# mindazhao/PWStableNet

Measured on AMD Instinct MI355X. Metric: stabilized frames/sec at 256x256 (netG fp32 + grid_sample), whole job, higher is better.
Workload: dtype f32

## Files before the change

### pwstablenet_amd/csrc/conv_ring_f32.hip

```cpp
#include "conv_common.h"

namespace pws {

typedef float rf_f32x2 __attribute__((ext_vector_type(2)));
typedef unsigned rf_u32x2 __attribute__((ext_vector_type(2)));

enum RingfMode {
    RF_K3S1 = 0,
    RF_CT4 = 1,
    RF_K3S2 = 2
};

struct RingfParams {
    const float *src_ptr[4];
    int src_c[4], src_ld[4];
    int nsrc;
    int N, H, W;
    int LH, LW;
    int OH, OW;
    int cout, cin_pad;
    const float *w;
    size_t w_bytes;
    const float *bias;
    int act;
    float *out;
    int out_ld;
    int tiles_x, tiles_y;
    unsigned ncob, ncls, nunits;
    int gpp;
};

template <int MODE_, int TH_, int R_, int NT_ = 2>
struct RfCfg {
    static constexpr int MODE = MODE_, TH = TH_, TW = 32, R = R_;
    static constexpr int NT = NT_, CO_UNIT = 32 * NT, WROWB = 128 * NT, WSL = 8 * NT;
    static_assert(NT == 1 || NT == 2, "output-channel blocks");
    static constexpr int KS = MODE == RF_K3S1 ? 3 : 2;
    static constexpr int TAPS = KS * KS;
    static constexpr int NPLANES = MODE == RF_K3S2 ? 4 : 1;
    static constexpr int NCLS = MODE == RF_CT4 ? 4 : 1;
    static constexpr int MWAVES = 8, LWAVES = 4, THREADS = 64 * (MWAVES + LWAVES);
    static_assert(TH == 16 || TH == 8, "tile");
    static constexpr int MT = TH / 8;
    static constexpr int IH = TH + KS - 1, IW = TW + KS - 1;
    static constexpr int CKG = 16;
    static constexpr int ROWB = CKG * 4;
    static constexpr int SPP = ROWB / 16;
    static constexpr int IN_SLOTS = IH * IW * SPP;
    static constexpr int IN_WI = (IN_SLOTS + 63) / 64;
    static constexpr int W_WI = TAPS * CKG * WROWB / 1024;
    static constexpr int NL = (IN_WI + W_WI + LWAVES - 1) / LWAVES;
    static constexpr int GROUP_BYTES = NL * LWAVES * 1024;
    static constexpr int W_OFF = IN_WI * 1024;
    static constexpr int LDS_BYTES = R * GROUP_BYTES;
    static constexpr int MIX_IT = IN_WI % LWAVES == 0 ? -1 : IN_WI / LWAVES;
    static_assert(LDS_BYTES <= 160 * 1024, "LDS");
    static_assert(R >= 2 && R <= 4, "ring depth");
    static_assert((R - 2) * NL <= 63, "vmcnt is 6 bits");
};

__device__ __forceinline__ void ringf_dma16(unsigned lds_addr, unsigned voff, __amdgpu_buffer_rsrc_t rsrc, unsigned soff) {
    unsigned keep;
    asm volatile("s_nop 4\n\ts_mov_b32 %0, m0\n\ts_mov_b32 m0, %1\n\ts_nop 0\n\tbuffer_load_dwordx4 %2, %3, %4 offen lds\n\ts_mov_b32 m0, %0"
                 : "=&s"(keep)
                 : "s"(lds_addr), "v"(voff), "s"(rsrc), "s"(soff));
}
__device__ __forceinline__ void ringf_dma16_m0(unsigned lds_addr, unsigned voff, __amdgpu_buffer_rsrc_t rsrc, unsigned soff) {
    asm volatile("s_nop 3\n\ts_mov_b32 m0, %0\n\ts_nop 0\n\tbuffer_load_dwordx4 %1, %2, %3 offen lds" ::"s"(lds_addr), "v"(voff), "s"(rsrc), "s"(soff));
}
template <int N>
__device__ __forceinline__ void ringf_wait_vmcnt() {
    asm volatile("s_waitcnt vmcnt(%0)" ::"n"(N) : "memory");
}
constexpr unsigned kRingfOob = 0x7ffffff0u;
__device__ __forceinline__ unsigned unif(unsigned v) { return __builtin_amdgcn_readfirstlane(v); }
__device__ __forceinline__ const char *unif(const char *ptr) {
    const unsigned long long a = reinterpret_cast<unsigned long long>(ptr);
    return reinterpret_cast<const char *>(((unsigned long long)unif((unsigned)(a >> 32)) << 32) | unif((unsigned)a));
}
template <class T>
__device__ __forceinline__ T selq4(const T (&a)[4], int i) {
    return i == 0 ? a[0] : (i == 1 ? a[1] : (i == 2 ? a[2] : a[3]));
}

struct RingfUnit {
    int n0, y0, x0, co0, py, px;
};
__device__ __forceinline__ RingfUnit ringf_unit(const RingfParams &p, unsigned u, int co_unit) {
    RingfUnit r;
    const unsigned cls = u % p.ncls, rest = u / p.ncls;
    const unsigned cob = rest % p.ncob, tile = rest / p.ncob;
    const unsigned tx = tile % (unsigned)p.tiles_x, t2 = tile / (unsigned)p.tiles_x;
    const unsigned ty = t2 % (unsigned)p.tiles_y;
    r.n0 = (int)(t2 / (unsigned)p.tiles_y);
    r.y0 = (int)ty, r.x0 = (int)tx, r.co0 = (int)cob * co_unit, r.py = (int)(cls >> 1), r.px = (int)(cls & 1);
    return r;
}

template <class C>
__global__ void __launch_bounds__(C::THREADS, 3) conv_ringf_kernel(const RingfParams p) {
    extern __shared__ __attribute__((aligned(16))) unsigned char lds[];
    const int tid = threadIdx.x, lane = tid & 63;
    const int wv = __builtin_amdgcn_readfirstlane(tid >> 6);
    const int l31 = lane & 31, hi = lane >> 5;

    const unsigned G = gridDim.x;
    const unsigned nxc = G < (unsigned)kXcds ? G : (unsigned)kXcds;
    const unsigned xcd = blockIdx.x % nxc, slot = blockIdx.x / nxc;
    const unsigned nx = G / nxc + (xcd < G % nxc ? 1u : 0u);
    const unsigned c_begin = (unsigned)((unsigned long long)xcd * p.nunits / nxc);
    const unsigned c_end = (unsigned)((unsigned long long)(xcd + 1) * p.nunits / nxc);
    if (c_begin + slot >= c_end) return;
    const unsigned u_begin = c_begin + slot, u_end = c_end, u_step = nx;
    const unsigned my_units = (u_end - u_begin + u_step - 1) / u_step;
    const int ngroups = C::NPLANES * p.gpp;
    const unsigned total = my_units * (unsigned)ngroups;

    if (wv >= C::MWAVES) {
        const int lw = wv - C::MWAVES;
        int ia[C::NL], ib[C::NL];
#pragma unroll
        for (int it = 0; it < C::NL; ++it) {
            const int wi = it * C::LWAVES + lw;
            const int j = wi * 64 + lane;
            if (wi < C::IN_WI) {
                const int q = j / C::SPP, sp = j % C::SPP;
                const int lx = q % C::IW, ly = q / C::IW;
                ia[it] = j < C::IN_SLOTS ? (ly << 10 | lx) : -1;
                ib[it] = (sp ^ ((lx >> 2) & 3)) * 16;
            } else if (wi < C::IN_WI + C::W_WI) {
                const int jj = j - C::IN_WI * 64;
                ia[it] = jj / C::WSL;
                ib[it] = jj % C::WSL;
            } else {
                ia[it] = -1, ib[it] = 0;
            }
        }
        const __amdgpu_buffer_rsrc_t rsrc_w = __builtin_amdgcn_make_buffer_rsrc(const_cast<float *>(p.w), 0, (int)p.w_bytes, 0x00020000);
        unsigned loc[C::NL], cv[C::NL];
        int loc_ld = -1;
#pragma unroll
        for (int it = 0; it < C::NL; ++it) loc[it] = kRingfOob, cv[it] = kRingfOob;
        unsigned issued = 0, dslot = 0;
        const bool mix_in = C::MIX_IT >= 0 && C::MIX_IT * C::LWAVES + lw < C::IN_WI;
        for (unsigned pu = u_begin; pu < u_end; pu += u_step) {
            const RingfUnit PU = ringf_unit(p, pu, C::CO_UNIT);
            for (int pplane = 0; pplane < C::NPLANES; ++pplane) {
                const int a = pplane >> 1, b = pplane & 1;
                int oy, ox;
                if constexpr (C::MODE == RF_K3S1) oy = PU.y0 * C::TH - 1, ox = PU.x0 * C::TW - 1;
                else if constexpr (C::MODE == RF_CT4) oy = PU.y0 * C::TH - (1 - PU.py), ox = PU.x0 * C::TW - (1 - PU.px);
                else oy = PU.y0 * C::TH - a, ox = PU.x0 * C::TW - b;
                unsigned d_sw = unif((unsigned)((size_t)PU.co0 * 4));
                const unsigned wplane = (unsigned)(p.cin_pad * p.cout * 4);
                const unsigned wstep = (unsigned)(C::CKG * p.cout * 4);
                for (int ps = 0; ps < p.nsrc; ++ps) {
                    const int ld = selq4(p.src_ld, ps), srcc = selq4(p.src_c, ps);
                    const size_t img = (size_t)p.H * p.W * ld * 4;
                    const char *base_in = unif(reinterpret_cast<const char *>(selq4(p.src_ptr, ps)) + (size_t)PU.n0 * img);
                    const __amdgpu_buffer_rsrc_t d_rin = __builtin_amdgcn_make_buffer_rsrc(const_cast<char *>(base_in), 0, (int)unif((unsigned)img), 0x00020000);
                    const unsigned ldb = (unsigned)ld * 4u;
                    const __amdgpu_buffer_rsrc_t d_rmix = __builtin_amdgcn_make_buffer_rsrc(
                        const_cast<char *>(unif(mix_in ? base_in : reinterpret_cast<const char *>(p.w))), 0,
                        (int)unif(mix_in ? (unsigned)img : (unsigned)p.w_bytes), 0x00020000);
                    constexpr int S = C::NPLANES == 4 ? 2 : 1;
                    if (ld != loc_ld) {
                        loc_ld = ld;
#pragma unroll
                        for (int it = 0; it < C::NL; ++it) {
                            if (it * C::LWAVES >= C::IN_WI) continue;
                            const int ly = ia[it] >> 10, lx = ia[it] & 0x3ff;
                            loc[it] = ia[it] >= 0 ? (unsigned)(S * ly * p.W + S * lx) * ldb + (unsigned)ib[it] : kRingfOob;
                        }
                    }
                    const int fy = S * oy + (S == 2 ? a : 0), fx = S * ox + (S == 2 ? b : 0);
                    const unsigned s_halo = unif((unsigned)((fy * p.W + fx) * (int)ldb));
                    const bool interior = fy >= 0 && fy + S * (C::IH - 1) < p.H && fx >= 0 && fx + S * (C::IW - 1) < p.W;
#pragma unroll
                    for (int it = 0; it < C::NL; ++it) {
                        const bool in_ct = (it + 1) * C::LWAVES <= C::IN_WI, w_ct = it * C::LWAVES >= C::IN_WI;
                        unsigned v_in = kRingfOob, v_w = kRingfOob;
                        if (!w_ct) {
                            v_in = loc[it] + s_halo;
                            if (!interior) {
                                const int ry = fy + S * (ia[it] >> 10), rx = fx + S * (ia[it] & 0x3ff);
                                v_in = (ia[it] >= 0 && ry >= 0 && ry < p.H && rx >= 0 && rx < p.W) ? v_in : kRingfOob;
                            }
                        }
                        if (!in_ct) {
                            const int t = ia[it] >> 4, k = ia[it] & 15;
                            int wt = t;
                            bool ok = ia[it] >= 0 && PU.co0 + ib[it] * 4 < p.cout;
                            const int ty = t >> 1, tx = t & 1;
                            if constexpr (C::MODE == RF_CT4) wt = (PU.py * 2 + PU.px) * 4 + t;
                            if constexpr (C::MODE == RF_K3S2) wt = (a ? 2 * ty : 1) * 3 + (b ? 2 * tx : 1), ok = ok && ty <= a && tx <= b;
                            v_w = ok ? (unsigned)wt * wplane + (unsigned)(k * p.cout + ib[it] * 4) * 4u : kRingfOob;
                        }
                        cv[it] = in_ct ? v_in : (w_ct ? v_w : (mix_in ? v_in : v_w));
                    }
                    unsigned d_sin = 0;
                    for (int pc0 = 0; pc0 < srcc; pc0 += C::CKG) {
                        if (issued >= (unsigned)(C::R - 1)) {
                            ringf_wait_vmcnt<(C::R - 2) * C::NL>();
                            __builtin_amdgcn_s_barrier();
                        }
                        const unsigned d_base = unif(dslot * (unsigned)C::GROUP_BYTES + (unsigned)(lw * 1024));
                        const unsigned d_smix = mix_in ? d_sin : d_sw;
                        unsigned keep;
                        asm volatile("s_nop 4\n\ts_mov_b32 %0, m0" : "=s"(keep));
#pragma unroll
                        for (int it = 0; it < C::NL; ++it) {
                            const bool in_ct = (it + 1) * C::LWAVES <= C::IN_WI, w_ct = it * C::LWAVES >= C::IN_WI;
                            const unsigned dst = d_base + (unsigned)(it * C::LWAVES * 1024);
                            if (in_ct) ringf_dma16_m0(dst, cv[it], d_rin, d_sin);
                            else if (w_ct) ringf_dma16_m0(dst, cv[it], rsrc_w, d_sw);
                            else ringf_dma16_m0(dst, cv[it], d_rmix, d_smix);
                        }
                        asm volatile("s_mov_b32 m0, %0" ::"s"(keep));
                        d_sin += (unsigned)(C::CKG * 4), d_sw += wstep;
                        ++issued;
                        dslot = dslot + 1 == (unsigned)C::R ? 0u : dslot + 1;
                    }
                }
            }
        }
        const unsigned rem = issued < (unsigned)(C::R - 1) ? issued : (unsigned)(C::R - 1);
        for (unsigned j = 0; j < rem; ++j) {
            const unsigned left = rem - 1 - j;
            if (left >= 2) ringf_wait_vmcnt<(C::R >= 4 ? 2 : 0) * C::NL>();
            else if (left == 1) ringf_wait_vmcnt<(C::R >= 3 ? 1 : 0) * C::NL>();
            else ringf_wait_vmcnt<0>();
            __builtin_amdgcn_s_barrier();
        }
        return;
    }

    int a_off[C::MT][C::KS];
#pragma unroll
    for (int mt = 0; mt < C::MT; ++mt)
#pragma unroll
        for (int dx = 0; dx < C::KS; ++dx) {
            const int lx = l31 + dx;
            a_off[mt][dx] = ((wv * C::MT + mt) * C::IW + lx) * C::ROWB + ((hi ^ ((lx >> 2) & 3)) << 4);
        }
    const int b_off = C::W_OFF + hi * 4 * C::WROWB + l31 * 4 * C::NT;

    f32x16 acc[C::MT][C::NT];
    unsigned cu = u_begin;
    int cg = 0, cplane = 0, cgp = 0, cbuf = 0;
    RingfUnit CU = ringf_unit(p, cu, C::CO_UNIT);

    for (unsigned s = 0; s < total; ++s) {
        asm volatile("" ::: "memory");
        __builtin_amdgcn_s_barrier();
        asm volatile("" ::: "memory");
        if (cg == 0) {
#pragma unroll
            for (int mt = 0; mt < C::MT; ++mt)
#pragma unroll
                for (int nt = 0; nt < C::NT; ++nt)
#pragma unroll
                    for (int r = 0; r < 16; ++r) acc[mt][nt][r] = 0.f;
        }
        unsigned tapmask = (1u << C::TAPS) - 1u;
        if constexpr (C::MODE == RF_K3S2) tapmask = (cplane >> 1) ? ((cplane & 1) ? 0xfu : 0x5u) : ((cplane & 1) ? 0x3u : 0x1u);
        const unsigned gb = (unsigned)(cbuf * C::GROUP_BYTES);
#pragma unroll
        for (int tap = 0; tap < C::TAPS; ++tap) {
            if constexpr (C::MODE == RF_K3S2) {
                if (!((tapmask >> tap) & 1u)) continue;
            }
            const int ty = tap / C::KS, tx = tap % C::KS;
#pragma unroll
            for (int t = 0; t < 2; ++t) {
                f32x4 a4[C::MT];
#pragma unroll
                for (int mt = 0; mt < C::MT; ++mt)
                    a4[mt] = *reinterpret_cast<const f32x4 *>(lds + gb + (unsigned)((a_off[mt][tx] ^ (t * 32)) + ty * C::IW * C::ROWB));
#pragma unroll
                for (int i = 0; i < 4; ++i) {
                    float bv[C::NT];
                    if constexpr (C::NT == 2) {
                        const rf_f32x2 b2 = *reinterpret_cast<const rf_f32x2 *>(lds + gb + (unsigned)(b_off + (tap * 16 + 8 * t + i) * C::WROWB));
                        bv[0] = b2[0], bv[1] = b2[1];
                    } else {
                        bv[0] = *reinterpret_cast<const float *>(lds + gb + (unsigned)(b_off + (tap * 16 + 8 * t + i) * C::WROWB));
                    }
#pragma unroll
                    for (int mt = 0; mt < C::MT; ++mt)
#pragma unroll
                        for (int nt = 0; nt < C::NT; ++nt)
                            acc[mt][nt] = __builtin_amdgcn_mfma_f32_32x32x2f32(a4[mt][i], bv[nt], acc[mt][nt], 0, 0, 0);
                }
            }
        }

        if (cg == ngroups - 1) {
            constexpr int SO = C::NCLS == 4 ? 2 : 1;
            const int co = CU.co0 + C::NT * l31;
            const bool co_ok = co < p.cout;
            float bs[C::NT];
#pragma unroll
            for (int nt = 0; nt < C::NT; ++nt) bs[nt] = (p.bias && co_ok) ? p.bias[co + nt] : 0.f;
            const size_t oimg = (size_t)p.OH * p.OW * p.out_ld;
            const __amdgpu_buffer_rsrc_t rsrc_o = __builtin_amdgcn_make_buffer_rsrc(p.out + (size_t)CU.n0 * oimg, 0, (int)(oimg * 4), 0x00020000);
            const unsigned pxb = (unsigned)(SO * p.out_ld * 4);
#pragma unroll
            for (int mt = 0; mt < C::MT; ++mt) {
                const int y = CU.y0 * C::TH + wv * C::MT + mt;
                const int oy = SO * y + (C::NCLS == 4 ? CU.py : 0);
                const int ox0 = SO * (CU.x0 * C::TW + 4 * hi) + (C::NCLS == 4 ? CU.px : 0);
                const unsigned vo = co_ok ? (unsigned)(((oy * p.OW + ox0) * p.out_ld + co) * 4) : kRingfOob;
#pragma unroll
                for (int r = 0; r < 16; ++r) {
                    const int soff = (int)(((r & 3) + 8 * (r >> 2)) * pxb);
                    if constexpr (C::NT == 2) {
                        const rf_f32x2 v = {act_apply(acc[mt][0][r] + bs[0], p.act), act_apply(acc[mt][1][r] + bs[1], p.act)};
                        __builtin_amdgcn_raw_buffer_store_b64(__builtin_bit_cast(rf_u32x2, v), rsrc_o, (int)vo, soff, 0);
                    } else {
                        __builtin_amdgcn_raw_buffer_store_b32(__builtin_bit_cast(unsigned, act_apply(acc[mt][0][r] + bs[0], p.act)), rsrc_o, (int)vo, soff, 0);
                    }
                }
            }
            cg = 0, cplane = 0, cgp = 0, cu += u_step;
            if (cu < u_end) CU = ringf_unit(p, cu, C::CO_UNIT);
        } else {
            ++cg;
            if (++cgp == p.gpp) cgp = 0, ++cplane;
        }
        cbuf = cbuf + 1 == C::R ? 0 : cbuf + 1;
    }
}

template <class C>
static int ringf_launch(RingfParams &rp, hipStream_t st) {
    static PerDeviceFlag attr_set_dev;
    bool &attr_set = attr_set_dev.cur();
    if (!attr_set) {
        hipError_t e = hipFuncSetAttribute(reinterpret_cast<const void *>(&conv_ringf_kernel<C>), hipFuncAttributeMaxDynamicSharedMemorySize,
                                           C::LDS_BYTES);
        if (e != hipSuccess) {
            set_error("hipFuncSetAttribute(conv_ringf_kernel, %d B LDS): %s", C::LDS_BYTES, hipGetErrorString(e));
            return PWS_EHIP;
        }
        attr_set = true;
    }
    static PerDeviceInt ncu_dev;
    int &ncu = ncu_dev.cur();
    if (ncu == 0) {
        int dev = 0;
        hipDeviceProp_t prop;
        ncu = (hipGetDevice(&dev) == hipSuccess && hipGetDeviceProperties(&prop, dev) == hipSuccess) ? prop.multiProcessorCount : 256;
    }
    rp.tiles_x = rp.LW / C::TW, rp.tiles_y = rp.LH / C::TH;
    rp.ncob = (unsigned)((rp.cout + C::CO_UNIT - 1) / C::CO_UNIT), rp.ncls = (unsigned)C::NCLS;
    rp.nunits = (unsigned)(rp.tiles_x * rp.tiles_y) * (unsigned)rp.N * rp.ncob * rp.ncls;
    int cin = 0;
    for (int s = 0; s < rp.nsrc; ++s) cin += rp.src_c[s];
    rp.gpp = cin / C::CKG;
    const unsigned grid = rp.nunits < (unsigned)ncu ? rp.nunits : (unsigned)ncu;
    hipLaunchKernelGGL((conv_ringf_kernel<C>), dim3(grid), dim3(C::THREADS), C::LDS_BYTES, st, rp);
    return check_launch("conv_ringf_kernel");
}

template <int MODE>
static int ringf_launch_tile(int th, int nt, RingfParams &rp, hipStream_t st) {
    constexpr int KS2 = MODE != RF_K3S1;
    if constexpr (MODE == RF_K3S2) {
        if (th == 8 && nt == 1) return ringf_launch<RfCfg<MODE, 8, 4, 1>>(rp, st);
    }
    if (th == 16) return ringf_launch<RfCfg<MODE, 16, KS2 ? 3 : 2>>(rp, st);
    return ringf_launch<RfCfg<MODE, 8, KS2 ? 4 : 2>>(rp, st);
}

int conv_ringf_try(int kind, const ConvKParams &kp, hipStream_t st, const ProfInfo &pi) {
    if (kp.io_bf16 || kp.ndst != 0 || g_experiment == 22) return 1;
    for (int s = 0; s < kp.nsrc; ++s)
        if (kp.src_ld[s] == 0 || kp.src_c[s] % 16 != 0 || kp.src_ld[s] % 4 != 0 || (reinterpret_cast<size_t>(kp.src_ptr[s]) & 15)) return 1;
    if (kp.LW % 32 != 0 || kp.LH % 8 != 0 || kp.cout % 4 != 0) return 1;
    if (kp.out_ld % 2 != 0 || (reinterpret_cast<size_t>(kp.out) & 7) || (size_t)kp.OH * kp.OW * kp.out_ld * 4 >= (1u << 31)) return 1;
    int mode, planes;
    if (kind == PWS_CONV_K3S1 || kind == PWS_CONVT_K3S1) mode = RF_K3S1, planes = 9;
    else if (kind == PWS_CONV_K3S2) mode = RF_K3S2, planes = 9;
    else if (kind == PWS_CONVT_K4S2) mode = RF_CT4, planes = 16;
    else return 1;
    for (int s = 0; s < kp.nsrc; ++s)
        if ((size_t)kp.H * kp.W * 4 * kp.src_ld[s] >= (1u << 31)) return 1;
    RingfParams rp{};
    for (int s = 0; s < 4; ++s) rp.src_ptr[s] = kp.src_ptr[s], rp.src_c[s] = kp.src_c[s], rp.src_ld[s] = kp.src_ld[s];
    rp.nsrc = kp.nsrc, rp.N = kp.N, rp.H = kp.H, rp.W = kp.W, rp.LH = kp.LH, rp.LW = kp.LW, rp.OH = kp.OH, rp.OW = kp.OW;
    rp.cout = kp.cout, rp.cin_pad = kp.cin_pad, rp.w = kp.w, rp.w_bytes = (size_t)planes * kp.cin_pad * kp.cout * 4;
    if (rp.w_bytes >= (1u << 31)) return 1;
    rp.bias = kp.bias, rp.act = kp.act, rp.out = kp.out, rp.out_ld = kp.out_ld;
    const long per256 = (long)kp.LW * kp.LH * kp.N / 256 * ((kp.cout + 63) / 64) * (mode == RF_CT4 ? 4 : 1);
    const long per256_32 = (long)kp.LW * kp.LH * kp.N / 256 * ((kp.cout + 31) / 32);
    int th, nt = 2;
    const bool forced = g_experiment == 23 || g_experiment == 24;
    if (g_experiment == 27 && mode == RF_K3S2) th = 8, nt = 1;
    else if (kp.LH % 16 == 0 && (per256 / 2 >= (mode == RF_K3S2 ? 256 : 512) || g_experiment == 24)) th = 16;
    else if (forced || (mode == RF_K3S2 && per256 >= 256)) th = 8;
    else if (mode == RF_K3S2 && per256_32 >= 256 && g_experiment != 26) th = 8, nt = 1;
    else return 1;
    if (mode == RF_CT4 && !forced) return 1;
    ProfScope prof(KID_CONV_RINGF, pi.flops, pi.bytes, st);
    switch (mode) {
    case RF_K3S1: return ringf_launch_tile<RF_K3S1>(th, nt, rp, st);
    case RF_CT4: return ringf_launch_tile<RF_CT4>(th, nt, rp, st);
    default: return ringf_launch_tile<RF_K3S2>(th, nt, rp, st);
    }
}

}
```

Measured before the change: 1981.

## Add half-size 4-wave ring conv variant for stride-2 convs to fit two blocks per CU

Adds a 4-MFMA-wave configuration of the ring-buffered fp32 conv kernel that halves the tile height, so two blocks share a CU. It becomes the default for stride-2 3x3 convs that previously used 8-row tiles, and the grid is sized to twice the CU count. The goal is more concurrent blocks per CU to hide DMA latency and balance small layers, at the cost of shallower rings and less weight reuse per block. It also adds ablation flags, driven by experiment numbers, that skip the DMA, MFMA or store phases for profiling.

New measurement: 2024, median of 6. 2.2% higher.

```diff
diff --git a/pwstablenet_amd/csrc/conv_ring_f32.hip b/pwstablenet_amd/csrc/conv_ring_f32.hip
--- a/pwstablenet_amd/csrc/conv_ring_f32.hip
+++ b/pwstablenet_amd/csrc/conv_ring_f32.hip
@@ -28,9 +28,10 @@
     int tiles_x, tiles_y;
     unsigned ncob, ncls, nunits;
     int gpp;
+    int ablate;
 };
 
-template <int MODE_, int TH_, int R_, int NT_ = 2>
+template <int MODE_, int TH_, int R_, int NT_ = 2, int MW_ = 8>
 struct RfCfg {
     static constexpr int MODE = MODE_, TH = TH_, TW = 32, R = R_;
     static constexpr int NT = NT_, CO_UNIT = 32 * NT, WROWB = 128 * NT, WSL = 8 * NT;
@@ -39,9 +40,11 @@
     static constexpr int TAPS = KS * KS;
     static constexpr int NPLANES = MODE == RF_K3S2 ? 4 : 1;
     static constexpr int NCLS = MODE == RF_CT4 ? 4 : 1;
-    static constexpr int MWAVES = 8, LWAVES = 4, THREADS = 64 * (MWAVES + LWAVES);
-    static_assert(TH == 16 || TH == 8, "tile");
-    static constexpr int MT = TH / 8;
+    static constexpr int MWAVES = MW_, LWAVES = 4, THREADS = 64 * (MWAVES + LWAVES);
+    static constexpr int WPC = MWAVES == 8 ? 1 : 2;
+    static constexpr int MINW = (THREADS / 64 * WPC + 3) / 4;
+    static_assert((MWAVES == 8 && (TH == 16 || TH == 8)) || (MWAVES == 4 && (TH == 8 || TH == 4)), "tile");
+    static constexpr int MT = TH / MWAVES;
     static constexpr int IH = TH + KS - 1, IW = TW + KS - 1;
     static constexpr int CKG = 16;
     static constexpr int ROWB = CKG * 4;
@@ -54,7 +57,7 @@
     static constexpr int W_OFF = IN_WI * 1024;
     static constexpr int LDS_BYTES = R * GROUP_BYTES;
     static constexpr int MIX_IT = IN_WI % LWAVES == 0 ? -1 : IN_WI / LWAVES;
-    static_assert(LDS_BYTES <= 160 * 1024, "LDS");
+    static_assert(LDS_BYTES * WPC <= 160 * 1024, "LDS");
     static_assert(R >= 2 && R <= 4, "ring depth");
     static_assert((R - 2) * NL <= 63, "vmcnt is 6 bits");
 };
@@ -98,7 +101,7 @@
 }
 
 template <class C>
-__global__ void __launch_bounds__(C::THREADS, 3) conv_ringf_kernel(const RingfParams p) {
+__global__ void __launch_bounds__(C::THREADS, C::MINW) conv_ringf_kernel(const RingfParams p) {
     extern __shared__ __attribute__((aligned(16))) unsigned char lds[];
     const int tid = threadIdx.x, lane = tid & 63;
     const int wv = __builtin_amdgcn_readfirstlane(tid >> 6);
@@ -206,17 +209,19 @@
                         }
                         const unsigned d_base = unif(dslot * (unsigned)C::GROUP_BYTES + (unsigned)(lw * 1024));
                         const unsigned d_smix = mix_in ? d_sin : d_sw;
-                        unsigned keep;
-                        asm volatile("s_nop 4\n\ts_mov_b32 %0, m0" : "=s"(keep));
-#pragma unroll
-                        for (int it = 0; it < C::NL; ++it) {
-                            const bool in_ct = (it + 1) * C::LWAVES <= C::IN_WI, w_ct = it * C::LWAVES >= C::IN_WI;
-                            const unsigned dst = d_base + (unsigned)(it * C::LWAVES * 1024);
-                            if (in_ct) ringf_dma16_m0(dst, cv[it], d_rin, d_sin);
-                            else if (w_ct) ringf_dma16_m0(dst, cv[it], rsrc_w, d_sw);
-                            else ringf_dma16_m0(dst, cv[it], d_rmix, d_smix);
+                        if (!(p.ablate & 2)) {
+                            unsigned keep;
+                            asm volatile("s_nop 4\n\ts_mov_b32 %0, m0" : "=s"(keep));
+#pragma unroll
+                            for (int it = 0; it < C::NL; ++it) {
+                                const bool in_ct = (it + 1) * C::LWAVES <= C::IN_WI, w_ct = it * C::LWAVES >= C::IN_WI;
+                                const unsigned dst = d_base + (unsigned)(it * C::LWAVES * 1024);
+                                if (in_ct) ringf_dma16_m0(dst, cv[it], d_rin, d_sin);
+                                else if (w_ct) ringf_dma16_m0(dst, cv[it], rsrc_w, d_sw);
+                                else ringf_dma16_m0(dst, cv[it], d_rmix, d_smix);
+                            }
+                            asm volatile("s_mov_b32 m0, %0" ::"s"(keep));
                         }
-                        asm volatile("s_mov_b32 m0, %0" ::"s"(keep));
                         d_sin += (unsigned)(C::CKG * 4), d_sw += wstep;
                         ++issued;
                         dslot = dslot + 1 == (unsigned)C::R ? 0u : dslot + 1;
@@ -266,7 +271,7 @@
         if constexpr (C::MODE == RF_K3S2) tapmask = (cplane >> 1) ? ((cplane & 1) ? 0xfu : 0x5u) : ((cplane & 1) ? 0x3u : 0x1u);
         const unsigned gb = (unsigned)(cbuf * C::GROUP_BYTES);
 #pragma unroll
-        for (int tap = 0; tap < C::TAPS; ++tap) {
+        for (int tap = 0; tap < C::TAPS && !(p.ablate & 1); ++tap) {
             if constexpr (C::MODE == RF_K3S2) {
                 if (!((tapmask >> tap) & 1u)) continue;
             }
@@ -307,6 +312,7 @@
             const unsigned pxb = (unsigned)(SO * p.out_ld * 4);
 #pragma unroll
             for (int mt = 0; mt < C::MT; ++mt) {
+                if (p.ablate & 4) break;
                 const int y = CU.y0 * C::TH + wv * C::MT + mt;
                 const int oy = SO * y + (C::NCLS == 4 ? CU.py : 0);
                 const int ox0 = SO * (CU.x0 * C::TW + 4 * hi) + (C::NCLS == 4 ? CU.px : 0);
@@ -358,15 +364,21 @@
     int cin = 0;
     for (int s = 0; s < rp.nsrc; ++s) cin += rp.src_c[s];
     rp.gpp = cin / C::CKG;
-    const unsigned grid = rp.nunits < (unsigned)ncu ? rp.nunits : (unsigned)ncu;
+    const unsigned slots = (unsigned)(ncu * C::WPC);
+    const unsigned grid = rp.nunits < slots ? rp.nunits : slots;
     hipLaunchKernelGGL((conv_ringf_kernel<C>), dim3(grid), dim3(C::THREADS), C::LDS_BYTES, st, rp);
     return check_launch("conv_ringf_kernel");
 }
 
 template <int MODE>
-static int ringf_launch_tile(int th, int nt, RingfParams &rp, hipStream_t st) {
+static int ringf_launch_tile(int th, int nt, bool half, RingfParams &rp, hipStream_t st) {
     constexpr int KS2 = MODE != RF_K3S1;
     if constexpr (MODE == RF_K3S2) {
+        if (half) {
+            if (th == 8) return ringf_launch<RfCfg<MODE, 8, 2, 2, 4>>(rp, st);
+            if (nt == 2) return ringf_launch<RfCfg<MODE, 4, 2, 2, 4>>(rp, st);
+            return ringf_launch<RfCfg<MODE, 4, 4, 1, 4>>(rp, st);
+        }
         if (th == 8 && nt == 1) return ringf_launch<RfCfg<MODE, 8, 4, 1>>(rp, st);
     }
     if (th == 16) return ringf_launch<RfCfg<MODE, 16, KS2 ? 3 : 2>>(rp, st);
@@ -402,12 +414,20 @@
     else if (mode == RF_K3S2 && per256_32 >= 256 && g_experiment != 26) th = 8, nt = 1;
     else return 1;
     if (mode == RF_CT4 && !forced) return 1;
+    bool half = mode == RF_K3S2 && th == 8;
+    if (mode == RF_K3S2 && g_experiment >= 2200 && g_experiment < 2248) {
+        const int v = (g_experiment - 2200) >> 4;
+        rp.ablate = (g_experiment - 2200) & 7;
+        if (v == 1) half = false;
+        else if (v == 2) half = true;
+    }
+    if (half) th /= 2;
     ProfScope prof(KID_CONV_RINGF, pi.flops, pi.bytes, st);
     switch (mode) {
-    case RF_K3S1: return ringf_launch_tile<RF_K3S1>(th, nt, rp, st);
-    case RF_CT4: return ringf_launch_tile<RF_CT4>(th, nt, rp, st);
-    default: return ringf_launch_tile<RF_K3S2>(th, nt, rp, st);
-    }
-}
-
-}
+    case RF_K3S1: return ringf_launch_tile<RF_K3S1>(th, nt, false, rp, st);
+    case RF_CT4: return ringf_launch_tile<RF_CT4>(th, nt, false, rp, st);
+    default: return ringf_launch_tile<RF_K3S2>(th, nt, half, rp, st);
+    }
+}
+
+}
```
